# ska-telescope/ska-sdp-screen-fitting

Measured on AMD Instinct MI355X. Metric: screen-slots/sec (ant×time×freq) + FITS-cube wall-clock, KL 256² screen, higher is better.
Workload: dtype f64

## Files before the change

### include/screenfit.h

```cpp
#ifndef SCREENFIT_H
#define SCREENFIT_H

#include <stddef.h>
#include <stdint.h>

#ifdef __cplusplus
extern "C" {
#endif

#define SF_OK 0
#define SF_EINVAL (-22)
#define SF_ENOMEM (-12)
#define SF_EIO (-5)
#define SF_ENODEV (-19)

#define SF_MAX_DIR 60
#define SF_MAX_FIT_DIR 128
#define SF_MAX_EVAL_DIR 128

#define SF_SCREEN_PHASE 0
#define SF_SCREEN_TEC 1
#define SF_SCREEN_AMPLITUDE 2

#define SF_EVAL_NAN_SCRUB 1u
// ... 48 lines not shown
#define SF_EVAL_KERNEL_LDS16 4
#define SF_EVAL_KERNEL_LDS8H 5
#define SF_EVAL_KERNEL_LDS16H 6
#define SF_EVAL_KERNEL_TILE3 7
#define SF_EVAL_KERNEL_SHB 8
#define SF_EVAL_KERNEL_WIDE 9
int sf_get_eval_kernel(sf_ctx* ctx, int gain, unsigned flags, int* kernel);
#define SF_EVAL_CONTRACTION_F64 0
#define SF_EVAL_CONTRACTION_I8_DIGITS 1
int sf_get_eval_contraction(sf_ctx* ctx, int gain, unsigned flags, int* contraction);
int sf_set_option(sf_ctx* ctx, int option, int value);
int sf_alloc(sf_ctx* ctx, size_t bytes, void** dev_ptr);
int sf_free(sf_ctx* ctx, void* dev_ptr);
int sf_copy_h2d(sf_ctx* ctx, void* dst_dev, const void* src_host, size_t bytes);
int sf_copy_d2h(sf_ctx* ctx, void* dst_host, const void* src_dev, size_t bytes);

int sf_set_basis(sf_ctx* ctx, const double* pp_host, int D, double r0,
                 double beta);
int sf_set_basis_wide(sf_ctx* ctx, const double* pp_host, int D, double r0,
                      double beta);
int sf_get_basis(sf_ctx* ctx, double* c_host, double* pinv_c_host,
                 double* u_host, double* eig_host);

int sf_set_piercepoints(sf_ctx* ctx, const double* pp_host, int D, double r0,
                        double beta);

int sf_kl_fit(sf_ctx* ctx, const double* phase, const float* weight, int T,
              int F, int A, const int* station_order_host,
              const sf_fit_params* params, double* coef, double* resid,
              float* w_out, int32_t* order_out);

int sf_get_fit_stats(sf_ctx* ctx, int* n_masks, int* n_general);

int sf_get_fit_pool(sf_ctx* ctx, uint64_t* masks_host, double* entries_host,
                    int max_masks, int* n_masks);

int sf_set_grid(sf_ctx* ctx, const double* x_host, int nx,
                const double* y_host, int ny);

int sf_kl_eval(sf_ctx* ctx, const double* coef, int64_t S, float* out,
               int64_t ring_slots, unsigned flags);

int sf_kl_eval_gain(sf_ctx* ctx, const double* coef_phase,
                    const double* coef_xx, const double* coef_yy, int64_t S,
                    float* out, int64_t ring_slots, unsigned flags);
int sf_kl_eval_sums(sf_ctx* ctx, const double* coef_phase,
                    const double* coef_xx, const double* coef_yy, int64_t S,
                    float* out, int64_t ring, unsigned flags,
                    uint32_t* slot_sums);

int sf_tess_fill(sf_ctx* ctx, const int32_t* labels, int nx, int ny,
                 const double* phase, const double* amp_xx,
                 const double* amp_yy, int D, int64_t S, float* out,
                 int64_t ring_slots, double smooth_pix, unsigned flags);

int sf_smooth(sf_ctx* ctx, float* cube, int nx, int ny, int64_t n_img,
              double smooth_pix, unsigned flags);

#ifdef __cplusplus
}
#endif
#endif
```

### ska-sdp-screen-fitting_amd/csrc/capi.hip

```cpp
#include <hip/hip_runtime.h>

#include <cmath>
#include <cstring>
#include <string>
#include <vector>

#include "sf_internal.h"

namespace sf {
static thread_local std::string g_last_error;
void set_error(const std::string& msg) { g_last_error = msg; }
}

using sf::set_error;

namespace {

int check_device(int device) {
  int n = 0;
  hipError_t e = hipGetDeviceCount(&n);
  if (e != hipSuccess || n == 0) {
    set_error("no HIP device available");
    return SF_ENODEV;
  }
// ... 131 lines not shown
    std::vector<uint32_t> mask((n_cu + 31) / 32, 0u);
    for (int c = 0; c < n_cu; ++c) mask[c >> 5] |= 1u << (c & 31);
    for (int k = 0; k < n_reserve; ++k) {
      const int c = reserve_cus[k];
      SF_REQUIRE(c >= 0 && c < n_cu, SF_EINVAL, "sf_stream_create: CU index out of range");
      mask[c >> 5] &= ~(1u << (c & 31));
    }
    SF_REQUIRE(n_reserve < n_cu, SF_EINVAL, "sf_stream_create: no CU left");
    SF_HIP(hipExtStreamCreateWithCUMask(&s, (uint32_t)mask.size(), mask.data()));
  }
  *stream = s;
  return SF_OK;
}

int sf_stream_destroy(sf_ctx* ctx, void* stream) {
  SF_REQUIRE(ctx && stream, SF_EINVAL, "sf_stream_destroy: bad argument");
  SF_HIP(hipSetDevice(ctx->device));
  SF_HIP(hipStreamDestroy(reinterpret_cast<hipStream_t>(stream)));
  return SF_OK;
}

int sf_set_option(sf_ctx* ctx, int option, int value) {
  SF_REQUIRE(ctx, SF_EINVAL, "sf_set_option: NULL context");
  switch (option) {
    case SF_OPT_FIT_GENERAL:
      ctx->force_general = value != 0;
      return SF_OK;
    case SF_OPT_EVAL_KERNEL:
      SF_REQUIRE(value >= SF_EVAL_KERNEL_AUTO && value <= SF_EVAL_KERNEL_WIDE,
                 SF_EINVAL, "sf_set_option: unknown evaluation kernel");
      ctx->eval_kernel = value;
      return SF_OK;
    case SF_OPT_FIT_PACK:
      ctx->fit_pack = value != 0;
      return SF_OK;
    case SF_OPT_FIT_LEAN:
      ctx->fit_lean = value != 0;
      return SF_OK;
    case SF_OPT_EVAL_KS_PAD:
      SF_REQUIRE(value >= 0 && value <= 3, SF_EINVAL,
                 "sf_set_option: k-step padding must be 0..3");
      ctx->eval_ks_pad = value;
      return SF_OK;
    case SF_OPT_EVAL_SLEEP:
      SF_REQUIRE(value >= 0 && value <= 1000, SF_EINVAL,
                 "sf_set_option: eval sleep must be 0..1000");
      ctx->eval_sleep = value;
      return SF_OK;
    case SF_OPT_EVAL_XCD_MAP:
      SF_REQUIRE(value >= -1 && value <= 1, SF_EINVAL,
                 "sf_set_option: XCD map must be -1, 0 or 1");
      ctx->eval_xcd_map = value;
      return SF_OK;
    case SF_OPT_EVAL_GROUPS:
      SF_REQUIRE(value >= 0 && value <= 256 && (value & (value - 1)) == 0,
                 SF_EINVAL, "sf_set_option: groups must be 0 or a power of two <= 256");
      ctx->eval_groups = value;
      return SF_OK;
    case SF_OPT_EVAL_BANDS:
      SF_REQUIRE(value >= 0 && value <= 128 && (value & (value - 1)) == 0,
                 SF_EINVAL, "sf_set_option: bands must be 0 or a power of two <= 128");
      ctx->eval_bands = value;
      return SF_OK;
    case SF_OPT_TESS_SLOTS:
      SF_REQUIRE(value >= 0 && value <= 256, SF_EINVAL,
                 "sf_set_option: tess slots must be 0..256");
      ctx->tess_slots = value;
// ... 232 lines not shown
               SF_EINVAL,
               "sf_kl_fit: reference station not in this shard and no "
               "ref_phase given");
  }
  for (int a = 0; a < A; ++a)
    SF_REQUIRE(st_order[a] >= 0, SF_EINVAL, "sf_kl_fit: negative order");
  SF_HIP(hipSetDevice(ctx->device));
  if (ctx->skip_cap < (size_t)F * A) {
    SF_TRY(dev_alloc(&ctx->d_skip, (size_t)F * A));
    ctx->skip_cap = (size_t)F * A;
  }
  if (ctx->st_order_cap < (size_t)A) {
    SF_TRY(dev_alloc(&ctx->d_st_order, (size_t)A));
    ctx->st_order_cap = (size_t)A;
  }
  SF_HIP(hipMemcpyAsync(ctx->d_st_order, st_order, sizeof(int) * A,
                        hipMemcpyHostToDevice, ctx->stream));
  return sf::launch_fit(ctx, phase, weight, T, F, A, p, coef, resid, w_out,
                        order_out);
}

int sf_get_fit_stats(sf_ctx* ctx, int* n_masks, int* n_general) {
  SF_REQUIRE(ctx, SF_EINVAL, "sf_get_fit_stats: NULL context");
  int c[4] = {0, 0, 0, 0};
  SF_HIP(hipSetDevice(ctx->device));
  SF_HIP(hipStreamSynchronize(ctx->stream));
  if (ctx->d_counters)
    SF_HIP(hipMemcpy(c, ctx->d_counters, sizeof(c), hipMemcpyDeviceToHost));
  if (n_masks) *n_masks = c[0];
  if (n_general) *n_general = c[2];
  return SF_OK;
}

int sf_get_fit_pool(sf_ctx* ctx, uint64_t* masks_host, double* entries_host,
                    int max_masks, int* n_masks) {
  SF_REQUIRE(ctx && n_masks && max_masks >= 0, SF_EINVAL, "sf_get_fit_pool: bad argument");
  SF_REQUIRE(max_masks == 0 || (masks_host && entries_host), SF_EINVAL,
             "sf_get_fit_pool: NULL output");
  SF_REQUIRE(!ctx->wide, SF_EINVAL,
             "sf_get_fit_pool: no mask pool above SF_MAX_DIR directions "
             "(sf_set_basis_wide: every flagged slot decomposes its own subset)");
  SF_HIP(hipSetDevice(ctx->device));
  SF_HIP(hipStreamSynchronize(ctx->stream));
  int c0 = 0;
  if (ctx->d_counters)
    SF_HIP(hipMemcpy(&c0, ctx->d_counters, sizeof(int), hipMemcpyDeviceToHost));
  const int n = ctx->pool_D == ctx->D && (size_t)c0 <= ctx->pool_cap ? c0 : 0;
  *n_masks = n;
  const int k = n < max_masks ? n : max_masks;
  if (k > 0) {
    const size_t entry = (size_t)ctx->D * ctx->D + ctx->D;
    SF_HIP(hipMemcpy(masks_host, ctx->d_pool_mask, k * sizeof(uint64_t),
                     hipMemcpyDeviceToHost));
    SF_HIP(hipMemcpy(entries_host, ctx->d_pool, k * entry * sizeof(double),
                     hipMemcpyDeviceToHost));
  }
  return SF_OK;
}

int sf_set_grid(sf_ctx* ctx, const double* x, int nx, const double* y,
                int ny) {
  SF_REQUIRE(ctx && ctx->D > 0, SF_EINVAL,
             "sf_set_grid: call sf_set_basis or sf_set_piercepoints first");
  SF_REQUIRE(x && y && nx >= 1 && ny >= 1, SF_EINVAL, "sf_set_grid: bad grid");
  for (int i = 0; i < nx; ++i)
    SF_REQUIRE(std::isfinite(x[i]), SF_EINVAL, "sf_set_grid: non-finite x coordinate");
// ... 203 lines not shown
```

### ska-sdp-screen-fitting_amd/csrc/kl_fit_fast.hip

```cpp
#include <hip/hip_runtime.h>

#include <algorithm>
#include <cmath>
#include <cstdlib>

#include "sf_internal.h"
#include "sf_wave.h"

namespace sf {

constexpr double kAtol = 1e-3;
constexpr size_t kLdsBytes = 160 * 1024;
constexpr double kTinyW = 1e-3 * 1.001;
constexpr unsigned long long kEmptyKey = 0ull;

__host__ __device__ inline int ldo(int n) { return n | 1; }

__device__ __forceinline__ unsigned long long mix64(unsigned long long x) {
  x ^= x >> 30;
  x *= 0xbf58476d1ce4e5b9ull;
  x ^= x >> 27;
  x *= 0x94d049bb133111ebull;
  x ^= x >> 31;
  return x;
// ... 18 lines not shown
    const unsigned long long k = keys[h];
    if (k == key) return h;
    if (k == kEmptyKey) return -1;
    h = (h + 1) & (cap - 1);
  }
  return -1;
}

__device__ __forceinline__ double phase_ref(const double* phase,
                                            const double* refph, int sub,
                                            int64_t s, int a, int A, int D,
                                            int d) {
  double v = phase[s * D + d];
  if (refph) v -= refph[(s / A) * D + d];
  else if (sub >= 0) v -= phase[(s + (sub - a)) * D + d];
  return v;
}

template <int GW>
__global__ __launch_bounds__(256) void kl_classify_kernel(
    const float* __restrict__ weight, int64_t S, int F, int A, int D,
    const int* __restrict__ st_order, const uint8_t* __restrict__ skip,
    int ref_skip, unsigned long long* __restrict__ keys, int cap,
    int* __restrict__ pos, uint8_t* __restrict__ cls,
    int* __restrict__ counters,
    double* __restrict__ coef, double* __restrict__ resid,
    float* __restrict__ w_out, int32_t* __restrict__ order_out) {
  constexpr int kPerWave = 64 / GW;
  const int l = lane();
  const int g = l / GW;
  const int d = l % GW;
  const int64_t s = ((int64_t)blockIdx.x * (blockDim.x / 64) + threadIdx.x / 64) *
                        kPerWave + g;
  const bool live = s < S && d < D;
  float x = 0.0f;
  if (live) {
    x = weight[s * D + d];
    w_out[s * D + d] = x;
  }
  const unsigned long long bm = __ballot(live && x > 0.0f);
  const unsigned long long bt = __ballot(live && x > 0.0f && (double)x <= kTinyW);
  const unsigned long long gmask = (GW == 64) ? ~0ull : ((1ull << GW) - 1ull);
  const unsigned long long mask = (bm >> (g * GW)) & gmask;
  const bool tiny = ((bt >> (g * GW)) & gmask) != 0ull;
  const float w_first = __shfl(x, g * GW + (mask ? __builtin_ctzll(mask) : 0));
  const unsigned long long bn = __ballot(live && x > 0.0f && x != w_first);
  const bool nonuniform = ((bn >> (g * GW)) & gmask) != 0ull;
  if (s >= S) return;
  const int a = (int)(s % A);
  const int f = (int)((s / A) % F);
  if (live && (a == ref_skip || skip[f * A + a])) {
    coef[s * D + d] = 0.0;
    resid[s * D + d] = 0.0;
  }
  if (d != 0) return;
  if (a == ref_skip || skip[f * A + a]) {
    cls[s] = 1;
    order_out[s] = 0;
    pos[s] = -2;
    return;
  }
  order_out[s] = st_order[a];
  if (tiny) atomicAdd(counters + 2, 1);
  else if (nonuniform) atomicAdd(counters + 4, 1);
  cls[s] = tiny ? 2 : 0;
  const unsigned long long full = (D == 64) ? ~0ull : ((1ull << D) - 1ull);
  if (mask == full) pos[s] = -1;
  else if (mask == 0ull) pos[s] = -2;
  else pos[s] = table_insert(keys, cap, mask);
}

__global__ __launch_bounds__(256) void kl_assign_kernel(
    const unsigned long long* __restrict__ keys, int cap, int* __restrict__ ids,
    unsigned long long* __restrict__ pool_mask, int pool_cap,
    int* __restrict__ counters, int D) {
  int lvl = 0;
  for (int i = blockIdx.x * blockDim.x + threadIdx.x; i - lane() < cap;
       i += gridDim.x * blockDim.x) {
    const unsigned long long k = i < cap ? keys[i] : kEmptyKey;
    const bool fresh = k != kEmptyKey && ids[i] < 0;
    const unsigned long long nb = __ballot(fresh);
// ... 359 lines not shown
        const double w = fabs(lam[k]);
        r2 += (w > v) || (w == v && k < l);
      }
      perm[r2] = l;
    }
    lds_sync();
    double* e = pool + (size_t)id * (D * D + D);
    if (l < m) {
      for (int r = 0; r < m; ++r) e[l * D + r] = U[l * ld + perm[r]];
      e[D * D + l] = lam[perm[l]];
    }
    if (l == 0) status[id] = 0;
    lds_sync();
  }
}

struct FastLds {
  const double* U;
  const double* C;
  int cld;
  const double* lam;
  double* Vs;
  double* lams;
  double* G;
  double* M;
  double* vec;
  double2* cs;
  int2* pr;
};

__host__ __device__ inline size_t fast_shared_bytes(int D, bool c_global) {
  return (size_t)((c_global ? 1 : 2) * D * ldo(D) + 64) * sizeof(double);
}
__host__ __device__ inline size_t fast_wave_bytes(int D, bool slow, bool lean = false) {
  if (lean) return (size_t)6 * 64 * sizeof(double);
  return (size_t)((slow ? 3 : 2) * D * ldo(D) + 64 + 6 * 64) * sizeof(double) +
         (slow ? 64 * sizeof(double2) + 96 * sizeof(int2) : 0);
}

struct Basis {
  int n;
  bool full;
  int ld;
  const double* U;
  const double* lam;
};

__device__ __noinline__ void nl_sincos(double x, double* s, double* c) { sincos(x, s, c); }
__device__ __noinline__ double nl_atan2(double y, double x) { return atan2(y, x); }
__device__ __noinline__ double nl_log10(double x) { return log10(x); }
__device__ __noinline__ double nl_pow(double x, double y) { return pow(x, y); }
__device__ __noinline__ double nl_log(double x) { return log(x); }
__device__ __noinline__ double nl_fmod(double x, double y) { return fmod(x, y); }

template <bool NI>
struct FitMath {
  static __device__ __forceinline__ void sin_cos(double x, double* s, double* c) {
    if constexpr (NI) nl_sincos(x, s, c); else sincos(x, s, c);
  }
  static __device__ __forceinline__ double arctan2(double y, double x) {
    if constexpr (NI) return nl_atan2(y, x); else return atan2(y, x);
  }
  static __device__ __forceinline__ double lg10(double x) {
    if constexpr (NI) return nl_log10(x); else return log10(x);
  }
  static __device__ __forceinline__ double power(double x, double y) {
    if constexpr (NI) return nl_pow(x, y); else return pow(x, y);
  }
  static __device__ __forceinline__ double ln(double x) {
    if constexpr (NI) return nl_log(x); else return log(x);
  }
  static __device__ __forceinline__ double mod(double x, double y) {
    if constexpr (NI) return nl_fmod(x, y); else return fmod(x, y);
  }
};

template <bool NI = false>
__device__ __forceinline__ double model_value(int screen_type, double x) {
  return screen_type == SF_SCREEN_AMPLITUDE ? FitMath<NI>::power(10.0, x) : x;
}

template <bool SLOW, int SPW, bool LEAN>
__device__ void fit_once(const FastLds& L, const Basis& B, int D, int ld,
                         int K, int screen_type, bool uniform, double wu,
                         double phi_p, double w_p, double phi_d, double w_d,
                         double& white_d, double& resid_d) {
#pragma clang fp contract(off)
  using G = Group<SPW>;
  using M = FitMath<!SLOW>;
  constexpr bool NI = !SLOW;
  constexpr int kMatVecUnroll = LEAN ? 4 : 1;
  const int l = G::lane();
  const int n = B.n;
  double* v0 = L.vec;
  double* v1 = L.vec + 64;
  double* v2 = L.vec + 128;
  double* v3 = L.vec + 192;
  double rc = 0.0, rs = 0.0;
  if (l < n) {
    if (screen_type == SF_SCREEN_PHASE) {
      double sn, cn;
      M::sin_cos(phi_p, &sn, &cn);
      rc = w_p * cn;
      rs = w_p * sn;
    } else if (screen_type == SF_SCREEN_AMPLITUDE) {
      rc = w_p * M::lg10(phi_p);
    } else {
      rc = w_p * phi_p;
    }
    v0[l] = rc;
    v1[l] = rs;
    v2[l] = w_p;
  }
  lds_sync();
  const bool tie2 = n == 2 && K == 1;
  double t_re = 0.0, t_im = 0.0;
  if (tie2) {
    const double w2 = v2[1];
    const double iw = w2 > kAtol ? 1.0 / w2 : 0.0;
    t_re = iw * v0[1];
    t_im = iw * v1[1];
  }
  double a1 = 0.0, a2 = 0.0;
  if (l < K) {
#pragma unroll kMatVecUnroll
    for (int p = 0; p < n; ++p) {
      const double u = B.U[p * B.ld + l];
      a1 += u * v0[p];
      a2 += u * v1[p];
    }
// ... 155 lines not shown
template <bool SLOW, int SPW, bool LEAN>
__global__ __launch_bounds__(256, SLOW ? 1 : SF_FIT_MINW) void kl_fit_pass_kernel(
    int it, int niter, int64_t S, int F, int A, int D,
    const double* __restrict__ phase, const double* __restrict__ refph,
    int ref_sub, const double* __restrict__ g_u, const double* __restrict__ g_c,
    const double* __restrict__ g_eig, const int* __restrict__ st_order,
    const uint8_t* __restrict__ cls, int* __restrict__ pos,
    const int* __restrict__ ids, unsigned long long* __restrict__ keys, int cap,
    const double* __restrict__ pool, int pool_cap, int* __restrict__ counters,
    int screen_type, double nsigma, int adjust_order, double* __restrict__ coef,
    double* __restrict__ resid, float* __restrict__ w_out,
    int32_t* __restrict__ order_out) {
#pragma clang fp contract(off)
  extern __shared__ double smem[];
  const int ld = ldo(D);
  using G = Group<SPW>;
  using M = FitMath<!SLOW>;
  constexpr bool NI = !SLOW;
  constexpr bool CG = SPW == 1;
  const int nwaves = blockDim.x / 64;
  const int nslots = nwaves * SPW;
  const int wv = (threadIdx.x / 64) * SPW + G::index();
  const int d = G::lane();
  double* sU = smem;
  double* sC = CG ? nullptr : sU + D * ld;
  double* sl = sU + (CG ? 1 : 2) * D * ld;
  for (int e = threadIdx.x; e < D * D; e += blockDim.x) {
    const int r = e / D, c = e % D;
    sU[r * ld + c] = g_u[e];
    if (!CG) sC[r * ld + c] = g_c[e];
  }
  for (int e = threadIdx.x; e < 64; e += blockDim.x) sl[e] = e < D ? g_eig[e] : 0.0;
  __syncthreads();
  FastLds L;
  L.U = sU;
  L.C = CG ? g_c : sC;
  L.cld = CG ? D : ld;
  L.lam = sl;
  double* wb = sl + 64 + (size_t)wv * (fast_wave_bytes(D, SLOW, LEAN) / sizeof(double));
  if (LEAN) {
    L.Vs = L.G = L.M = L.lams = nullptr;
    L.vec = wb;
    L.cs = nullptr;
    L.pr = nullptr;
  } else {
    L.Vs = wb;
    L.G = wb + D * ld;
    L.M = L.G + D * ld;
    L.lams = (SLOW ? L.M + D * ld : L.G + D * ld);
    L.vec = L.lams + 64;
    L.cs = reinterpret_cast<double2*>(L.vec + 6 * 64);
    L.pr = reinterpret_cast<int2*>(L.cs + 64);
  }
  const uint8_t want = SLOW ? 2 : 0;

  for (int64_t s = (int64_t)blockIdx.x * nslots + wv; s < S;
       s += (int64_t)gridDim.x * nslots) {
    if (SLOW && cls[s] != want) continue;
    const uint8_t cl = SLOW ? want : cls[s];
    const int a = (int)(s % A);
    const int p0 = pos[s];
    const int64_t base = s * D;
    double phi_d = 0.0, w_d = 0.0, white_d = 0.0, resid_d = 0.0;
    if (d < D) {
      phi_d = phase_ref(phase, refph, ref_sub, s, a, A, D, d);
      w_d = (double)w_out[base + d];
      white_d = it == 0 ? 0.0 : coef[base + d];
      resid_d = it == 0 ? 0.0 : resid[base + d];
    }
    double order = (double)order_out[s];
    const double station_order = (double)st_order[a];
    if (cl != want) continue;
    int id = -1;
    if (p0 >= 0) {
      id = ids[p0];
      if (id < 0 || id >= pool_cap) {
        if (d == 0) atomicOr(counters + 3, 1);
        continue;
      }
    } else if (p0 == -3) {
      if (d == 0) atomicOr(counters + 3, 2);
      continue;
    }
    const bool unfl = (d < D) && (w_d > 0.0);
    const unsigned long long um = G::ballot(unfl);
    const int n_unfl = __popcll(um);

    Basis B;
    B.n = n_unfl;
    B.full = (n_unfl == D);
    B.ld = ld;
    if (B.full) {
      B.U = L.U;
      B.lam = L.lam;
    } else if (n_unfl > 0) {
      const double* e = pool + (size_t)id * (D * D + D);
      if (LEAN) {
        B.U = e;
        B.ld = D;
        B.lam = e + D * D;
      } else {
        for (int r = 0; r < n_unfl; ++r)
          if (d < n_unfl) L.Vs[r * ld + d] = e[r * D + d];
        if (d < n_unfl) L.lams[d] = e[D * D + d];
        lds_sync();
        B.U = L.Vs;
        B.lam = L.lams;
      }
    }
    double phi_p = 0.0, w_p = 0.0;
    {
      double* v4 = L.vec + 256;
      double* v5 = L.vec + 320;
      if (unfl) {
        const int p = G::rank(um);
        v4[p] = phi_d;
        v5[p] = w_d;
      }
      lds_sync();
      if (d < n_unfl) {
        phi_p = v4[d];
        w_p = v5[d];
      }
      lds_sync();
    }
    const double wmax = G::max(unfl ? w_d : -INFINITY);
    const double wmin = -G::max(unfl ? -w_d : -INFINITY);
    const bool uniform = (wmax == wmin);
    if (LEAN && n_unfl > 0 && !uniform) {
      if (d == 0) atomicOr(counters + 3, 4);
      continue;
    }

    if (n_unfl > 0) {
      if (order > n_unfl - 1) order = n_unfl - 1;
      if (it == 0) {
        fit_once<SLOW, SPW, LEAN>(L, B, D, ld, (int)order, screen_type, uniform, wmin,
                       phi_p, w_p, phi_d, w_d, white_d, resid_d);
      } else if (adjust_order) {
        bool hit_upper = false, hit_lower = false, hit_upper2 = false,
             hit_lower2 = false;
        double sign = 1.0, prev_redchi2 = 0.0;
        for (int oi = 0; oi < 4; ++oi) {
          if (oi > 0)
            fit_once<SLOW, SPW, LEAN>(L, B, D, ld, (int)order, screen_type, uniform, wmin,
                           phi_p, w_p, phi_d, w_d, white_d, resid_d);
// ... 234 lines not shown
    const size_t shm = (size_t)2 * subset_rows(D) * subset_ld(D) * sizeof(double) +
                       64 * sizeof(double2) + 96 * sizeof(int2) +
                       128 * sizeof(int);
    const int blocks = n_new < 8192 ? n_new : 8192;
    const int nw = ctx->fit_eig_waves > 0 ? ctx->fit_eig_waves : kEigWavesDefault;
#define SF_LAUNCH_EIG(NW)                                                              \
  do {                                                                                 \
    if (shm > 64 * 1024)                                                               \
      SF_HIP(hipFuncSetAttribute(reinterpret_cast<const void*>(&kl_subset_eig_kernel<NW>), \
                                 hipFuncAttributeMaxDynamicSharedMemorySize, (int)shm)); \
    hipLaunchKernelGGL(kl_subset_eig_kernel<NW>, dim3(blocks), dim3(64 * NW), shm,     \
                       ctx->stream, ctx->d_c, D, ctx->d_pool_mask, (int)ctx->pool_cap, \
                       ctx->d_counters, ctx->d_pool, done);                            \
  } while (0)
    switch (nw) {
      case 1: SF_LAUNCH_EIG(1); break;
      case 2: SF_LAUNCH_EIG(2); break;
      case 4: SF_LAUNCH_EIG(4); break;
      default: SF_LAUNCH_EIG(3); break;
    }
#undef SF_LAUNCH_EIG
    SF_HIP(hipGetLastError());
  }
  return SF_OK;
}

template <bool SLOW, int SPW, bool LEAN>
static int launch_pass_spw(sf_ctx* ctx, int it, const sf_fit_params* p,
                           const RefSpec& r, int64_t S, int F, int A,
                           const double* phase, double* coef, double* resid,
                           float* w_out, int32_t* order_out) {
  const int D = ctx->D;
  const size_t shared = fast_shared_bytes(D, SPW == 1);
  const size_t slot = fast_wave_bytes(D, SLOW, LEAN);
  int nw = 1, best = 0;
  for (int k = 1; k <= 4; ++k) {
    const size_t per_wg = shared + (size_t)k * SPW * slot;
    if (per_wg > kLdsBytes) break;
    const int waves = k * (int)(kLdsBytes / per_wg);
    if (waves > best) {
      best = waves;
      nw = k;
    }
  }
  const size_t shm = shared + (size_t)nw * SPW * slot;
  if (shm > 64 * 1024)
    SF_HIP(hipFuncSetAttribute(
        reinterpret_cast<const void*>(&kl_fit_pass_kernel<SLOW, SPW, LEAN>),
        hipFuncAttributeMaxDynamicSharedMemorySize, (int)shm));
  int64_t blocks = (S + nw * SPW - 1) / (nw * SPW);
  if (blocks > 16384) blocks = 16384;
  hipLaunchKernelGGL((kl_fit_pass_kernel<SLOW, SPW, LEAN>), dim3((unsigned)blocks),
                     dim3(64 * nw), shm, ctx->stream, it, p->niter, S, F, A, D,
                     phase, r.refph, r.sub, ctx->d_u, ctx->d_c, ctx->d_eig,
                     ctx->d_st_order, ctx->d_class, ctx->d_pos, ctx->d_ids,
                     ctx->d_keys, (int)ctx->table_cap, ctx->d_pool,
                     (int)ctx->pool_cap, ctx->d_counters, p->screen_type,
                     p->nsigma, p->adjust_order, coef, resid, w_out, order_out);
  SF_HIP(hipGetLastError());
  return SF_OK;
}

template <bool SLOW>
static int launch_pass(sf_ctx* ctx, int it, const sf_fit_params* p,
                       const RefSpec& r, int64_t S, int F, int A,
                       const double* phase, double* coef, double* resid,
                       float* w_out, int32_t* order_out, bool lean) {
  const bool pack = !SLOW && ctx->D <= 32 && ctx->fit_pack;
  if (!SLOW && lean && ctx->fit_lean) {
    if (pack)
      return launch_pass_spw<false, 2, true>(ctx, it, p, r, S, F, A, phase, coef,
                                             resid, w_out, order_out);
    return launch_pass_spw<false, 1, true>(ctx, it, p, r, S, F, A, phase, coef,
                                           resid, w_out, order_out);
  }
  if (pack)
    return launch_pass_spw<SLOW, 2, false>(ctx, it, p, r, S, F, A, phase, coef,
                                           resid, w_out, order_out);
  return launch_pass_spw<SLOW, 1, false>(ctx, it, p, r, S, F, A, phase, coef, resid,
                                         w_out, order_out);
}

int launch_block_sigma(sf_ctx* ctx, int T, int F, int A, const double* phase,
                       const RefSpec& r, int screen_type, const double* resid,
                       const float* w_out) {
  hipLaunchKernelGGL(kl_block_sigma_kernel, dim3(F * A), dim3(256), 0,
                     ctx->stream, T, F, A, ctx->D, phase, r.refph, r.sub,
                     ctx->d_skip, r.skip, screen_type, resid, w_out,
                     ctx->d_sigma);
  SF_HIP(hipGetLastError());
  return SF_OK;
}

int launch_fit(sf_ctx* ctx, const double* phase, const float* weight, int T,
               int F, int A, const sf_fit_params* p, double* coef,
               double* resid, float* w_out, int32_t* order_out) {
  if (ctx->wide)
    return launch_fit_wide(ctx, phase, weight, T, F, A, p, coef, resid, w_out,
                           order_out);
  const int D = ctx->D;
  const int64_t S = (int64_t)T * F * A;
  const RefSpec r = ref_spec(p, A);
  SF_TRYF(launch_skip(ctx, phase, weight, T, F, A, r));

  static const char* env = std::getenv("SCREENFIT_FIT");
  if (ctx->force_general || (env && env[0] == 'g')) {
    if (p->screen_type == SF_SCREEN_AMPLITUDE ||
        (p->niter > 1 && p->screen_type != SF_SCREEN_PHASE)) {
      set_error("the general fit kernel handles phase (any niter) and tec (niter 1) only");
      return SF_EINVAL;
    }
    return launch_fit_general(ctx, nullptr, nullptr, S, phase, weight, T, F, A,
                              p, r, coef, resid, w_out, order_out);
  }
  if (!resid) {
    SF_TRYF(grow(&ctx->d_scratch, ctx->scratch_cap, (size_t)S * D));
    resid = ctx->d_scratch;
  }
  if (!w_out || !order_out) {
    size_t wc = 0, oc = 0;
    if (ctx->d_wscratch) (void)hipFree(ctx->d_wscratch);
    if (ctx->d_oscratch) (void)hipFree(ctx->d_oscratch);
    ctx->d_wscratch = nullptr;
    ctx->d_oscratch = nullptr;
    SF_TRYF(grow(&ctx->d_wscratch, wc, (size_t)S * D));
    SF_TRYF(grow(&ctx->d_oscratch, oc, (size_t)S));
    if (!w_out) w_out = ctx->d_wscratch;
    if (!order_out) order_out = ctx->d_oscratch;
  }
// ... 7 lines not shown
    SF_TRYF(grow(&ctx->d_class, c3, (size_t)S));
    ctx->slot_cap = (size_t)S;
  }
  if (ctx->sigma_cap < (size_t)F * A) {
    size_t c = 0;
    if (ctx->d_sigma) (void)hipFree(ctx->d_sigma);
    ctx->d_sigma = nullptr;
    SF_TRYF(grow(&ctx->d_sigma, c, (size_t)F * A));
    ctx->sigma_cap = (size_t)F * A;
  }
  const size_t tcap = next_pow2((size_t)(2 * p->niter + 2) * (size_t)S + 64);
  if (ctx->table_cap < tcap) {
    size_t c1 = 0, c2 = 0;
    if (ctx->d_keys) (void)hipFree(ctx->d_keys);
    if (ctx->d_ids) (void)hipFree(ctx->d_ids);
    ctx->d_keys = nullptr;
    ctx->d_ids = nullptr;
    SF_TRYF(grow(&ctx->d_keys, c1, tcap));
    SF_TRYF(grow(&ctx->d_ids, c2, tcap));
    ctx->table_cap = tcap;
  }
  if (!ctx->d_counters) {
    size_t c = 0;
    SF_TRYF(grow(&ctx->d_counters, c, 8));
  }
  SF_TRYF(ensure_pool(ctx, 1024));
  const int cap = (int)ctx->table_cap;
  SF_HIP(hipMemsetAsync(ctx->d_keys, 0, ctx->table_cap * sizeof(unsigned long long),
                        ctx->stream));
  SF_HIP(hipMemsetAsync(ctx->d_ids, 0xff, ctx->table_cap * sizeof(int), ctx->stream));
  SF_HIP(hipMemsetAsync(ctx->d_counters, 0, 8 * sizeof(int), ctx->stream));

  {
    const int gw = D <= 8 ? 8 : D <= 16 ? 16 : D <= 32 ? 32 : 64;
    const int64_t per_block = 4 * (64 / gw);
    const dim3 grid((unsigned)((S + per_block - 1) / per_block));
#define SF_CLASSIFY(W)                                                          \
  hipLaunchKernelGGL(kl_classify_kernel<W>, grid, dim3(256), 0, ctx->stream,    \
                     weight, S, F, A, D, ctx->d_st_order, ctx->d_skip, r.skip,  \
                     ctx->d_keys, cap, ctx->d_pos, ctx->d_class,               \
                     ctx->d_counters, coef, resid, w_out, order_out)
    switch (gw) {
      case 8: SF_CLASSIFY(8); break;
      case 16: SF_CLASSIFY(16); break;
      case 32: SF_CLASSIFY(32); break;
      default: SF_CLASSIFY(64); break;
    }
#undef SF_CLASSIFY
    SF_HIP(hipGetLastError());
  }

  const bool block_flags = p->screen_type != SF_SCREEN_PHASE;
  for (int it = 0; it < p->niter; ++it) {
    int n_slow = 0, n_nonuniform = 0;
    SF_TRYF(number_and_decompose(ctx, &n_slow, &n_nonuniform));
    SF_TRYF(launch_pass<false>(ctx, it, p, r, S, F, A, phase, coef, resid,
                               w_out, order_out, n_nonuniform == 0));
    if (n_slow > 0)
      SF_TRYF(launch_pass<true>(ctx, it, p, r, S, F, A, phase, coef, resid,
                                w_out, order_out, false));
    if (block_flags && it + 1 < p->niter) {
      SF_TRYF(launch_block_sigma(ctx, T, F, A, phase, r, p->screen_type, resid,
                                 w_out));
      hipLaunchKernelGGL(kl_block_flag_kernel, dim3((unsigned)((S + 255) / 256)),
                         dim3(256), 0, ctx->stream, S, F, A, D, phase, r.refph,
                         r.sub, ctx->d_class, p->screen_type, p->nsigma,
                         ctx->d_sigma, resid, w_out, ctx->d_keys, cap,
                         ctx->d_pos);
      SF_HIP(hipGetLastError());
    }
  }
  int err = 0;
  SF_HIP(hipMemcpyAsync(&err, ctx->d_counters + 3, sizeof(int),
                        hipMemcpyDeviceToHost, ctx->stream));
  SF_HIP(hipStreamSynchronize(ctx->stream));
  SF_REQUIRE((err & 3) == 0, SF_EIO, "sf_kl_fit: internal mask table overflow");
  SF_REQUIRE((err & 4) == 0, SF_EIO,
// ... 10 lines not shown
```

### ska-sdp-screen-fitting_amd/csrc/sf_internal.h

```cpp
#pragma once

#include <hip/hip_runtime.h>

#include <cstdint>
#include <string>

#include "screenfit.h"

namespace sf {

void set_error(const std::string& msg);

#define SF_HIP(call)                                                        \
  do {                                                                      \
    hipError_t e_ = (call);                                                 \
    if (e_ != hipSuccess) {                                                 \
      ::sf::set_error(std::string(#call) + ": " + hipGetErrorString(e_));   \
      return SF_EIO;                                                        \
    }                                                                       \
  } while (0)

#define SF_REQUIRE(cond, code, msg) \
  do {                              \
    if (!(cond)) {                  \
// ... 87 lines not shown
  size_t pool_status_cap = 0;
  int pool_D = 0;
  int* d_pos = nullptr;
  uint8_t* d_class = nullptr;
  double* d_sigma = nullptr;
  size_t sigma_cap = 0;
  size_t slot_cap = 0;
  int* d_counters = nullptr;
  double* d_scratch = nullptr;
  size_t scratch_cap = 0;
  float* d_wscratch = nullptr;
  int32_t* d_oscratch = nullptr;
  double* d_gw = nullptr;
  size_t gw_cap = 0;
  double gw_sigma = -1.0;
  float* d_trash = nullptr;
  float* d_smooth = nullptr;
  size_t smooth_cap = 0;
  float* d_tess_tab = nullptr;
  size_t tess_tab_cap = 0;
  int force_general = 0;
  int eval_kernel = SF_EVAL_KERNEL_AUTO;
  int64_t eval_max_blocks = 0;
  int eval_ks_pad = 0;
  int eval_sleep = 0;
  int eval_xcd_map = -1;
  int eval_groups = 0;
  int eval_bands = 0;
  int tess_slots = 0;
  int tess_waves = 0;
  int tess_tile = 0;
  int tess_box = -1;
  int fit_pack = 1;
  int fit_lean = 1;
};

namespace sf {
constexpr int kEvalMaxKS = 15;
constexpr int kEvalWideMaxKS = SF_MAX_EVAL_DIR / 4;
inline bool eval_int_applies(const sf_ctx* ctx, bool gain, unsigned flags,
                             bool out_aligned16) {
  return !gain && ctx->dig_ok && ctx->d_cdig && ctx->eval_int != 0 &&
         (flags & SF_EVAL_FAST_SINCOS) && ctx->n_pix % 4 == 0 && out_aligned16 &&
         ctx->ksteps >= 12 && ctx->ksteps <= kEvalMaxKS;
}

struct RefSpec {
  int sub = -1;
  const double* refph = nullptr;
  int skip = -1;
};
RefSpec ref_spec(const sf_fit_params* p, int A);
int launch_skip(sf_ctx* ctx, const double* phase, const float* weight, int T,
                int F, int A, const RefSpec& r);
int launch_fit_general(sf_ctx* ctx, const int* slot_list, const int* n_list,
                       int64_t max_slots, const double* phase,
                       const float* weight, int T, int F, int A,
                       const sf_fit_params* p, const RefSpec& r, double* coef,
                       double* resid, float* w_out, int32_t* order_out);
int launch_basis(sf_ctx* ctx);
int launch_block_sigma(sf_ctx* ctx, int T, int F, int A, const double* phase,
                       const RefSpec& r, int screen_type, const double* resid,
                       const float* w_out);
int launch_basis_wide(sf_ctx* ctx);
int launch_fit_wide(sf_ctx* ctx, const double* phase, const float* weight,
                    int T, int F, int A, const sf_fit_params* p, double* coef,
// ... 27 lines not shown
```

### ska-sdp-screen-fitting_amd/csrc/sf_wave.h

```cpp
#pragma once

#include <hip/hip_runtime.h>

namespace sf {

__device__ __forceinline__ int lane() { return __lane_id(); }

__device__ __forceinline__ void lds_sync() {
  asm volatile("s_waitcnt lgkmcnt(0)" ::: "memory");
}

__device__ __forceinline__ double wave_sum(double v) {
#pragma unroll
  for (int o = 32; o > 0; o >>= 1) v += __shfl_xor(v, o, 64);
  return v;
}

__device__ __forceinline__ double wave_max(double v) {
#pragma unroll
  for (int o = 32; o > 0; o >>= 1) v = fmax(v, __shfl_xor(v, o, 64));
  return v;
}

__device__ __forceinline__ double bcast(double v, int src) {
  return __shfl(v, src, 64);
}

template <int SPW>
struct Group {
  static constexpr int kWidth = 64 / SPW;
  __device__ static int lane() { return __lane_id() & (kWidth - 1); }
  __device__ static int first() { return __lane_id() & ~(kWidth - 1); }
  __device__ static int index() { return __lane_id() / kWidth; }
  __device__ static double sum(double v) {
#pragma unroll
    for (int o = kWidth / 2; o > 0; o >>= 1) v += __shfl_xor(v, o, 64);
    return v;
  }
  __device__ static double max(double v) {
#pragma unroll
    for (int o = kWidth / 2; o > 0; o >>= 1) v = fmax(v, __shfl_xor(v, o, 64));
    return v;
  }
  __device__ static double bcast(double v, int src) {
    return __shfl(v, first() + src, 64);
  }
  __device__ static unsigned long long ballot(bool x) {
    const unsigned long long m = __ballot(x);
    if (SPW == 1) return m;
    return (m >> first()) & ((1ull << kWidth) - 1);
  }
  __device__ static bool any(bool x) { return ballot(x) != 0ull; }
  __device__ static int rank(unsigned long long m) {
    if (SPW == 1)
      return __builtin_amdgcn_mbcnt_hi((uint32_t)(m >> 32),
                                       __builtin_amdgcn_mbcnt_lo((uint32_t)m, 0));
    return __popcll(m & ((1ull << lane()) - 1));
  }
};

__device__ __forceinline__ int rr_partner(int i, int r, int m) {
  const int mm = m - 1;
  if (i == mm) return r;
  if (i == r) return mm;
  int p = 2 * r - i;
  if (p < 0) p += mm;
  if (p >= mm) p -= mm;
  return p;
}

__device__ inline int wave_jacobi(double* a, double* v, double2* cs, int2* pr,
                                  int n, int ld, int max_sweeps) {
#pragma clang fp contract(off)
  const int i = lane();
// ... 285 lines not shown
```

### ska-sdp-screen-fitting_amd/ska_sdp_screen_fitting_amd/_lib.py

```python

import contextlib
import ctypes
import os
import threading

import numpy as np

_HERE = os.path.dirname(os.path.abspath(__file__))
LIB_PATH = os.environ.get("SCREENFIT_LIB", os.path.join(_HERE, "libscreenfit.so"))

SF_SCREEN_PHASE = 0
SF_SCREEN_TEC = 1
SF_SCREEN_AMPLITUDE = 2
SF_EVAL_NAN_SCRUB = 1
SF_EVAL_FAST_SINCOS = 1 << 8
SF_EVAL_NT_STORES = 1 << 9
SF_EVAL_BIG_ENDIAN = 1 << 10
SF_MAX_DIR = 60
SF_MAX_FIT_DIR = 128
SF_MAX_EVAL_DIR = 128
SF_OPT_FIT_GENERAL = 1
SF_OPT_EVAL_KERNEL = 2
SF_OPT_EVAL_MAX_BLOCKS = 3
SF_OPT_FIT_PACK = 4
# ... 4 lines not shown
SF_OPT_EVAL_BANDS = 9
SF_OPT_FIT_LEAN = 10
SF_OPT_TESS_SLOTS = 11
SF_OPT_TESS_WAVES = 12
SF_OPT_TESS_TILE = 13
SF_OPT_TESS_BOX = 14
SF_OPT_EVAL_INT = 15
SF_OPT_EVAL_WG_WAVES = 16
SF_OPT_FIT_EIG_WAVES = 17
SF_OPT_FIT_SUBSET_DELETION = 18
SF_EVAL_KERNEL_AUTO = 0
SF_EVAL_KERNEL_TILE = 1
SF_EVAL_KERNEL_LDS4 = 2
SF_EVAL_KERNEL_LDS8 = 3
SF_EVAL_KERNEL_LDS16 = 4
SF_EVAL_KERNEL_LDS8H = 5
SF_EVAL_KERNEL_LDS16H = 6
SF_EVAL_KERNEL_TILE3 = 7
SF_EVAL_KERNEL_SHB = 8
SF_EVAL_KERNEL_WIDE = 9
EVAL_KERNEL_NAMES = {SF_EVAL_KERNEL_TILE: "kl_eval_kernel",
                     SF_EVAL_KERNEL_LDS4: "kl_eval_lds_kernel<4 waves>",
                     SF_EVAL_KERNEL_LDS8: "kl_eval_lds_kernel<8 waves>",
                     SF_EVAL_KERNEL_LDS16: "kl_eval_lds_kernel<16 waves>",
                     SF_EVAL_KERNEL_LDS8H: "kl_eval_lds_kernel<8 waves, 2 tiles>",
                     SF_EVAL_KERNEL_LDS16H: "kl_eval_lds_kernel<16 waves, 2 tiles>",
                     SF_EVAL_KERNEL_TILE3: "kl_eval_kernel<3 waves/SIMD>",
                     SF_EVAL_KERNEL_SHB: "kl_eval_kernel<Cpix in LDS>",
                     SF_EVAL_KERNEL_WIDE: "kl_eval_wide_kernel"}

EXPORTED = (
    "sf_version", "sf_last_error", "sf_create", "sf_destroy", "sf_set_stream",
    "sf_synchronize", "sf_set_option", "sf_get_eval_kernel", "sf_get_eval_contraction", "sf_alloc", "sf_free", "sf_copy_h2d", "sf_copy_d2h",
    "sf_set_basis", "sf_set_basis_wide", "sf_set_piercepoints", "sf_get_basis", "sf_kl_fit", "sf_get_fit_stats", "sf_get_fit_pool",
    "sf_stream_create", "sf_stream_destroy", "sf_device_cus",
    "sf_set_grid", "sf_kl_eval", "sf_kl_eval_gain", "sf_kl_eval_sums",
    "sf_tess_fill", "sf_smooth",
)


_identity = {}


def library_identity(path=None):
    import hashlib
    p = os.path.realpath(path or LIB_PATH)
    if p not in _identity:
        h = hashlib.sha256()
        with open(p, "rb") as fh:
            for blk in iter(lambda: fh.read(1 << 20), b""):
                h.update(blk)
        _identity[p] = {"sha16": h.hexdigest()[:16], "bytes": os.path.getsize(p)}
    return dict(_identity[p])


class ScreenFitError(RuntimeError):
    """Raised for any failure of the HIP library (including its absence)."""


class FitParams(ctypes.Structure):
    _fields_ = [("screen_type", ctypes.c_int), ("niter", ctypes.c_int),
                ("nsigma", ctypes.c_double), ("adjust_order", ctypes.c_int),
                ("ref_ant", ctypes.c_int), ("ant_offset", ctypes.c_int),
                ("ref_phase", ctypes.c_void_p)]


_lib = None
# ... 6 lines not shown
        if _lib is not None and path is None:
            return _lib
        p = path or LIB_PATH
        if not os.path.exists(p):
            raise ScreenFitError(
                f"libscreenfit.so not found at {p}: build it with "
                "`make -C ska-sdp-screen-fitting_amd/csrc` (or "
                "__graft_entry__.build()); there is no CPU fallback")
        lib = ctypes.CDLL(p)
        vp, ip, c_int, c_dbl = (ctypes.c_void_p, ctypes.POINTER(ctypes.c_int),
                                ctypes.c_int, ctypes.c_double)
        i64 = ctypes.c_int64
        sig = {
            "sf_version": ([], ctypes.c_char_p),
            "sf_last_error": ([], ctypes.c_char_p),
            "sf_create": ([c_int, ctypes.POINTER(vp)], c_int),
            "sf_destroy": ([vp], c_int),
            "sf_set_stream": ([vp, vp], c_int),
            "sf_synchronize": ([vp], c_int),
            "sf_set_option": ([vp, c_int, c_int], c_int),
            "sf_get_eval_kernel": ([vp, c_int, ctypes.c_uint, ip], c_int),
            "sf_get_eval_contraction": ([vp, c_int, ctypes.c_uint, ip], c_int),
            "sf_alloc": ([vp, ctypes.c_size_t, ctypes.POINTER(vp)], c_int),
            "sf_free": ([vp, vp], c_int),
            "sf_copy_h2d": ([vp, vp, vp, ctypes.c_size_t], c_int),
            "sf_copy_d2h": ([vp, vp, vp, ctypes.c_size_t], c_int),
            "sf_set_basis": ([vp, vp, c_int, c_dbl, c_dbl], c_int),
            "sf_set_basis_wide": ([vp, vp, c_int, c_dbl, c_dbl], c_int),
            "sf_set_piercepoints": ([vp, vp, c_int, c_dbl, c_dbl], c_int),
            "sf_get_basis": ([vp, vp, vp, vp, vp], c_int),
            "sf_kl_fit": ([vp, vp, vp, c_int, c_int, c_int, ip,
                           ctypes.POINTER(FitParams), vp, vp, vp, vp], c_int),
            "sf_get_fit_stats": ([vp, ip, ip], c_int),
            "sf_get_fit_pool": ([vp, vp, vp, c_int, ip], c_int),
            "sf_set_grid": ([vp, vp, c_int, vp, c_int], c_int),
            "sf_kl_eval": ([vp, vp, i64, vp, i64, ctypes.c_uint], c_int),
            "sf_stream_create": ([vp, ctypes.POINTER(c_int), c_int,
                                  ctypes.POINTER(vp)], c_int),
            "sf_stream_destroy": ([vp, vp], c_int),
            "sf_device_cus": ([vp, ctypes.POINTER(c_int)], c_int),
            "sf_kl_eval_gain": ([vp, vp, vp, vp, i64, vp, i64, ctypes.c_uint],
                                c_int),
            "sf_kl_eval_sums": ([vp, vp, vp, vp, i64, vp, i64, ctypes.c_uint, vp],
                                c_int),
            "sf_tess_fill": ([vp, vp, c_int, c_int, vp, vp, vp, c_int, i64, vp,
                              i64, c_dbl, ctypes.c_uint], c_int),
            "sf_smooth": ([vp, vp, c_int, c_int, i64, c_dbl, ctypes.c_uint], c_int),
        }
        for name, (args, res) in sig.items():
            fn = getattr(lib, name)
            fn.argtypes = args
            fn.restype = res
        if path is None:
            _lib = lib
        return lib


def _check(rc, what):
    if rc != 0:
        msg = load_library().sf_last_error().decode(errors="replace")
        raise ScreenFitError(f"{what} failed ({rc}): {msg}")


_TORCH_DTYPES = {np.float64: "torch.float64", np.float32: "torch.float32",
                 np.int32: "torch.int32", np.int64: "torch.int64"}

# ... 104 lines not shown
        c, pinv, u = (np.empty((D, D)) for _ in range(3))
        eig = np.empty(D)
        _check(self.lib.sf_get_basis(self.h, c.ctypes.data, pinv.ctypes.data,
                                     u.ctypes.data, eig.ctypes.data),
               "sf_get_basis")
        return c, pinv, u, eig

    def fit(self, phase, weight, T, F, A, station_order, screen_type=0,
            niter=2, nsigma=5.0, adjust_order=True, ref_ant=-1, coef=None,
            resid=None, w_out=None, order_out=None, ant_offset=0,
            ref_phase=None):
        so = np.ascontiguousarray(station_order, dtype=np.int32)
        if so.shape != (A,):
            raise ValueError(f"station_order: shape {so.shape}, expected ({A},)")
        n = int(T) * int(F) * int(A) * self.D
        prm = FitParams(int(screen_type), int(niter), float(nsigma),
                        int(bool(adjust_order)), int(ref_ant), int(ant_offset),
                        self._dev(ref_phase, np.float64, int(T) * int(F) * self.D,
                             "ref_phase"))
        _check(self.lib.sf_kl_fit(
            self.h, self._dev(phase, np.float64, n, "phase"),
            self._dev(weight, np.float32, n, "weight"), int(T), int(F), int(A),
            so.ctypes.data_as(ctypes.POINTER(ctypes.c_int)),
            ctypes.byref(prm), self._dev(coef, np.float64, n, "coef"),
            self._dev(resid, np.float64, n, "resid"),
            self._dev(w_out, np.float32, n, "w_out"),
            self._dev(order_out, np.int32, n // max(self.D, 1), "order_out")),
            "sf_kl_fit")

    def fit_stats(self):
        nm, ng = ctypes.c_int(), ctypes.c_int()
        _check(self.lib.sf_get_fit_stats(self.h, ctypes.byref(nm), ctypes.byref(ng)),
               "sf_get_fit_stats")
        return {"n_masks": nm.value, "n_general": ng.value}

    def fit_pool(self):
        n = ctypes.c_int(0)
        _check(self.lib.sf_get_fit_pool(self.h, None, None, 0, ctypes.byref(n)),
               "sf_get_fit_pool")
        D = self.D
        masks = np.zeros(n.value, np.uint64)
        ent = np.zeros((n.value, D * D + D))
        if n.value:
            _check(self.lib.sf_get_fit_pool(self.h, masks.ctypes.data, ent.ctypes.data,
                                            n.value, ctypes.byref(n)), "sf_get_fit_pool")
        order = np.argsort(masks, kind="stable")
        masks, ent = masks[order], ent[order]
        for k, m in enumerate(masks):
            n = bin(int(m)).count("1")
            u = ent[k, :D * D].reshape(D, D)
            u[n:, :] = 0.0
            u[:, n:] = 0.0
            ent[k, D * D + n:] = 0.0
        return masks, ent

    def set_grid(self, x, y):
        x = np.ascontiguousarray(x, dtype=np.float64)
        y = np.ascontiguousarray(y, dtype=np.float64)
        _check(self.lib.sf_set_grid(self.h, x.ctypes.data, x.size,
                                    y.ctypes.data, y.size), "sf_set_grid")
        self.grid = (x.size, y.size)

    def _out_numel(self, S, ring):
        nx, ny = self.grid if self.grid else (0, 0)
        return min(int(S), ring) * 4 * nx * ny

    def eval(self, coef, S, out, ring_slots=None,
# ... 110 lines not shown
```

Baseline: 6.335 million.

## Pack more fit slots per wavefront with D-dependent group widths

```diff
diff --git a/include/screenfit.h b/include/screenfit.h
--- a/include/screenfit.h
+++ b/include/screenfit.h
@@ -104,6 +104,8 @@
 
 int sf_get_fit_stats(sf_ctx* ctx, int* n_masks, int* n_general);
 
+int sf_get_fit_pack(sf_ctx* ctx, int* slots_per_wave);
+
 int sf_get_fit_pool(sf_ctx* ctx, uint64_t* masks_host, double* entries_host,
                     int max_masks, int* n_masks);
 
diff --git a/ska-sdp-screen-fitting_amd/csrc/capi.hip b/ska-sdp-screen-fitting_amd/csrc/capi.hip
--- a/ska-sdp-screen-fitting_amd/csrc/capi.hip
+++ b/ska-sdp-screen-fitting_amd/csrc/capi.hip
@@ -187,7 +187,9 @@
       ctx->eval_kernel = value;
       return SF_OK;
     case SF_OPT_FIT_PACK:
-      ctx->fit_pack = value != 0;
+      SF_REQUIRE(value >= 0 && value <= 2, SF_EINVAL,
+                 "sf_set_option: fit packing must be 0, 1 or 2");
+      ctx->fit_pack = value;
       return SF_OK;
     case SF_OPT_FIT_LEAN:
       ctx->fit_lean = value != 0;
@@ -486,6 +488,12 @@
   return SF_OK;
 }
 
+int sf_get_fit_pack(sf_ctx* ctx, int* slots_per_wave) {
+  SF_REQUIRE(ctx && slots_per_wave, SF_EINVAL, "sf_get_fit_pack: bad argument");
+  *slots_per_wave = ctx->fit_spw_last;
+  return SF_OK;
+}
+
 int sf_get_fit_pool(sf_ctx* ctx, uint64_t* masks_host, double* entries_host,
                     int max_masks, int* n_masks) {
   SF_REQUIRE(ctx && n_masks && max_masks >= 0, SF_EINVAL, "sf_get_fit_pool: bad argument");
diff --git a/ska-sdp-screen-fitting_amd/csrc/kl_fit_fast.hip b/ska-sdp-screen-fitting_amd/csrc/kl_fit_fast.hip
--- a/ska-sdp-screen-fitting_amd/csrc/kl_fit_fast.hip
+++ b/ska-sdp-screen-fitting_amd/csrc/kl_fit_fast.hip
@@ -74,7 +74,7 @@
   const int d = l % GW;
   const int64_t s = ((int64_t)blockIdx.x * (blockDim.x / 64) + threadIdx.x / 64) *
                         kPerWave + g;
-  const bool live = s < S && d < D;
+  const bool live = g < kPerWave && s < S && d < D;
   float x = 0.0f;
   if (live) {
     x = weight[s * D + d];
@@ -85,10 +85,11 @@
   const unsigned long long gmask = (GW == 64) ? ~0ull : ((1ull << GW) - 1ull);
   const unsigned long long mask = (bm >> (g * GW)) & gmask;
   const bool tiny = ((bt >> (g * GW)) & gmask) != 0ull;
-  const float w_first = __shfl(x, g * GW + (mask ? __builtin_ctzll(mask) : 0));
+  const float w_first =
+      __shfl(x, g < kPerWave ? g * GW + (mask ? __builtin_ctzll(mask) : 0) : l);
   const unsigned long long bn = __ballot(live && x > 0.0f && x != w_first);
   const bool nonuniform = ((bn >> (g * GW)) & gmask) != 0ull;
-  if (s >= S) return;
+  if (g >= kPerWave || s >= S) return;
   const int a = (int)(s % A);
   const int f = (int)((s / A) % F);
   if (live && (a == ref_skip || skip[f * A + a])) {
@@ -514,9 +515,14 @@
 __host__ __device__ inline size_t fast_shared_bytes(int D, bool c_global) {
   return (size_t)((c_global ? 1 : 2) * D * ldo(D) + 64) * sizeof(double);
 }
-__host__ __device__ inline size_t fast_wave_bytes(int D, bool slow, bool lean = false) {
-  if (lean) return (size_t)6 * 64 * sizeof(double);
-  return (size_t)((slow ? 3 : 2) * D * ldo(D) + 64 + 6 * 64) * sizeof(double) +
+__host__ __device__ constexpr int fast_vec_len(int spw) {
+  return spw == 1 ? 64 : spw <= 3 ? 32 : 64 / spw;
+}
+__host__ __device__ inline size_t fast_wave_bytes(int D, bool slow, bool lean = false,
+                                                  int vlen = 64) {
+  const int vecs = 6 * vlen + (vlen < 64 ? 2 : 0);
+  if (lean) return (size_t)vecs * sizeof(double);
+  return (size_t)((slow ? 3 : 2) * D * ldo(D) + 64 + vecs) * sizeof(double) +
          (slow ? 64 * sizeof(double2) + 96 * sizeof(int2) : 0);
 }
 
@@ -574,10 +580,11 @@
   constexpr int kMatVecUnroll = LEAN ? 4 : 1;
   const int l = G::lane();
   const int n = B.n;
+  constexpr int VL = fast_vec_len(SPW);
   double* v0 = L.vec;
-  double* v1 = L.vec + 64;
-  double* v2 = L.vec + 128;
-  double* v3 = L.vec + 192;
+  double* v1 = L.vec + VL;
+  double* v2 = L.vec + 2 * VL;
+  double* v3 = L.vec + 3 * VL;
   double rc = 0.0, rs = 0.0;
   if (l < n) {
     if (screen_type == SF_SCREEN_PHASE) {
@@ -799,12 +806,14 @@
   }
   for (int e = threadIdx.x; e < 64; e += blockDim.x) sl[e] = e < D ? g_eig[e] : 0.0;
   __syncthreads();
+  if (G::index() >= SPW) return;
   FastLds L;
   L.U = sU;
   L.C = CG ? g_c : sC;
   L.cld = CG ? D : ld;
   L.lam = sl;
-  double* wb = sl + 64 + (size_t)wv * (fast_wave_bytes(D, SLOW, LEAN) / sizeof(double));
+  constexpr int VL = fast_vec_len(SPW);
+  double* wb = sl + 64 + (size_t)wv * (fast_wave_bytes(D, SLOW, LEAN, VL) / sizeof(double));
   if (LEAN) {
     L.Vs = L.G = L.M = L.lams = nullptr;
     L.vec = wb;
@@ -816,7 +825,7 @@
     L.M = L.G + D * ld;
     L.lams = (SLOW ? L.M + D * ld : L.G + D * ld);
     L.vec = L.lams + 64;
-    L.cs = reinterpret_cast<double2*>(L.vec + 6 * 64);
+    L.cs = reinterpret_cast<double2*>(L.vec + 6 * VL);
     L.pr = reinterpret_cast<int2*>(L.cs + 64);
   }
   const uint8_t want = SLOW ? 2 : 0;
@@ -877,8 +886,8 @@
     }
     double phi_p = 0.0, w_p = 0.0;
     {
-      double* v4 = L.vec + 256;
-      double* v5 = L.vec + 320;
+      double* v4 = L.vec + 4 * VL;
+      double* v5 = L.vec + 5 * VL;
       if (unfl) {
         const int p = G::rank(um);
         v4[p] = phi_d;
@@ -1179,7 +1188,7 @@
                            float* w_out, int32_t* order_out) {
   const int D = ctx->D;
   const size_t shared = fast_shared_bytes(D, SPW == 1);
-  const size_t slot = fast_wave_bytes(D, SLOW, LEAN);
+  const size_t slot = fast_wave_bytes(D, SLOW, LEAN, fast_vec_len(SPW));
   int nw = 1, best = 0;
   for (int k = 1; k <= 4; ++k) {
     const size_t per_wg = shared + (size_t)k * SPW * slot;
@@ -1208,24 +1217,45 @@
   return SF_OK;
 }
 
+static int fit_slots_per_wave(const sf_ctx* ctx) {
+  const int D = ctx->D;
+  if (ctx->fit_pack == 0 || D > 32) return 1;
+  if (ctx->fit_pack == 2) return 2;
+  return D <= 8 ? 8 : D <= 16 ? 4 : D <= 21 ? 3 : 2;
+}
+
 template <bool SLOW>
 static int launch_pass(sf_ctx* ctx, int it, const sf_fit_params* p,
                        const RefSpec& r, int64_t S, int F, int A,
                        const double* phase, double* coef, double* resid,
                        float* w_out, int32_t* order_out, bool lean) {
-  const bool pack = !SLOW && ctx->D <= 32 && ctx->fit_pack;
-  if (!SLOW && lean && ctx->fit_lean) {
-    if (pack)
-      return launch_pass_spw<false, 2, true>(ctx, it, p, r, S, F, A, phase, coef,
-                                             resid, w_out, order_out);
-    return launch_pass_spw<false, 1, true>(ctx, it, p, r, S, F, A, phase, coef,
-                                           resid, w_out, order_out);
-  }
-  if (pack)
-    return launch_pass_spw<SLOW, 2, false>(ctx, it, p, r, S, F, A, phase, coef,
-                                           resid, w_out, order_out);
-  return launch_pass_spw<SLOW, 1, false>(ctx, it, p, r, S, F, A, phase, coef, resid,
-                                         w_out, order_out);
+#define SF_PASS(SPW, LEAN)                                                      \
+  return launch_pass_spw<SLOW, SPW, LEAN>(ctx, it, p, r, S, F, A, phase, coef, \
+                                          resid, w_out, order_out)
+  if constexpr (SLOW) {
+    SF_PASS(1, false);
+  } else {
+    int spw = fit_slots_per_wave(ctx);
+    const bool lean_pass = lean && ctx->fit_lean;
+    if (!lean_pass && spw == 3) spw = 2;
+    ctx->fit_spw_last = spw;
+    if (lean_pass) {
+      switch (spw) {
+        case 8: SF_PASS(8, true);
+        case 4: SF_PASS(4, true);
+        case 3: SF_PASS(3, true);
+        case 2: SF_PASS(2, true);
+        default: SF_PASS(1, true);
+      }
+    }
+    switch (spw) {
+      case 8: SF_PASS(8, false);
+      case 4: SF_PASS(4, false);
+      case 2: SF_PASS(2, false);
+      default: SF_PASS(1, false);
+    }
+  }
+#undef SF_PASS
 }
 
 int launch_block_sigma(sf_ctx* ctx, int T, int F, int A, const double* phase,
@@ -1242,6 +1272,7 @@
 int launch_fit(sf_ctx* ctx, const double* phase, const float* weight, int T,
                int F, int A, const sf_fit_params* p, double* coef,
                double* resid, float* w_out, int32_t* order_out) {
+  ctx->fit_spw_last = 1;
   if (ctx->wide)
     return launch_fit_wide(ctx, phase, weight, T, F, A, p, coef, resid, w_out,
                            order_out);
@@ -1315,7 +1346,8 @@
   SF_HIP(hipMemsetAsync(ctx->d_counters, 0, 8 * sizeof(int), ctx->stream));
 
   {
-    const int gw = D <= 8 ? 8 : D <= 16 ? 16 : D <= 32 ? 32 : 64;
+    const int gw = D <= 8 ? 8 : D <= 16 ? 16
+                 : fit_slots_per_wave(ctx) == 3 ? 21 : D <= 32 ? 32 : 64;
     const int64_t per_block = 4 * (64 / gw);
     const dim3 grid((unsigned)((S + per_block - 1) / per_block));
 #define SF_CLASSIFY(W)                                                          \
@@ -1326,6 +1358,7 @@
     switch (gw) {
       case 8: SF_CLASSIFY(8); break;
       case 16: SF_CLASSIFY(16); break;
+      case 21: SF_CLASSIFY(21); break;
       case 32: SF_CLASSIFY(32); break;
       default: SF_CLASSIFY(64); break;
     }
diff --git a/ska-sdp-screen-fitting_amd/csrc/sf_internal.h b/ska-sdp-screen-fitting_amd/csrc/sf_internal.h
--- a/ska-sdp-screen-fitting_amd/csrc/sf_internal.h
+++ b/ska-sdp-screen-fitting_amd/csrc/sf_internal.h
@@ -143,6 +143,7 @@
   int tess_tile = 0;
   int tess_box = -1;
   int fit_pack = 1;
+  int fit_spw_last = 1;
   int fit_lean = 1;
 };
 
diff --git a/ska-sdp-screen-fitting_amd/csrc/sf_wave.h b/ska-sdp-screen-fitting_amd/csrc/sf_wave.h
--- a/ska-sdp-screen-fitting_amd/csrc/sf_wave.h
+++ b/ska-sdp-screen-fitting_amd/csrc/sf_wave.h
@@ -29,17 +29,49 @@
 template <int SPW>
 struct Group {
   static constexpr int kWidth = 64 / SPW;
-  __device__ static int lane() { return __lane_id() & (kWidth - 1); }
-  __device__ static int first() { return __lane_id() & ~(kWidth - 1); }
+  static constexpr bool kPow2 = (kWidth & (kWidth - 1)) == 0;
+  static_assert(SPW == 1 || kWidth <= 32, "groups are at most half a wave");
+  static_assert(kPow2 || kWidth > 16, "the partner rule needs p ^ 16 < kWidth");
   __device__ static int index() { return __lane_id() / kWidth; }
+  __device__ static int first() {
+    return kPow2 ? (__lane_id() & ~(kWidth - 1)) : index() * kWidth;
+  }
+  __device__ static int lane() {
+    return kPow2 ? (__lane_id() & (kWidth - 1)) : __lane_id() - first();
+  }
+  __device__ static int partner(int o) {
+    int p = lane() ^ o;
+    if (p >= kWidth) p ^= 16;
+    return first() + p;
+  }
   __device__ static double sum(double v) {
-#pragma unroll
-    for (int o = kWidth / 2; o > 0; o >>= 1) v += __shfl_xor(v, o, 64);
+    if (kPow2) {
+#pragma unroll
+      for (int o = 16; o >= kWidth && SPW > 1; o >>= 1) v += 0.0;
+#pragma unroll
+      for (int o = kWidth / 2; o > 0; o >>= 1) v += __shfl_xor(v, o, 64);
+    } else {
+      const int l = lane();
+      const double x = __shfl(v, first() + ((l ^ 16) < kWidth ? (l ^ 16) : l), 64);
+      v += (l ^ 16) < kWidth ? x : 0.0;
+#pragma unroll
+      for (int o = 8; o > 0; o >>= 1) v += __shfl(v, partner(o), 64);
+    }
     return v;
   }
   __device__ static double max(double v) {
-#pragma unroll
-    for (int o = kWidth / 2; o > 0; o >>= 1) v = fmax(v, __shfl_xor(v, o, 64));
+    if (kPow2) {
+#pragma unroll
+      for (int o = 16; o >= kWidth && SPW > 1; o >>= 1) v = fmax(v, -INFINITY);
+#pragma unroll
+      for (int o = kWidth / 2; o > 0; o >>= 1) v = fmax(v, __shfl_xor(v, o, 64));
+    } else {
+      const int l = lane();
+      const double x = __shfl(v, first() + ((l ^ 16) < kWidth ? (l ^ 16) : l), 64);
+      v = fmax(v, (l ^ 16) < kWidth ? x : -INFINITY);
+#pragma unroll
+      for (int o = 8; o > 0; o >>= 1) v = fmax(v, __shfl(v, partner(o), 64));
+    }
     return v;
   }
   __device__ static double bcast(double v, int src) {
diff --git a/ska-sdp-screen-fitting_amd/ska_sdp_screen_fitting_amd/_lib.py b/ska-sdp-screen-fitting_amd/ska_sdp_screen_fitting_amd/_lib.py
--- a/ska-sdp-screen-fitting_amd/ska_sdp_screen_fitting_amd/_lib.py
+++ b/ska-sdp-screen-fitting_amd/ska_sdp_screen_fitting_amd/_lib.py
@@ -60,7 +60,7 @@
 EXPORTED = (
     "sf_version", "sf_last_error", "sf_create", "sf_destroy", "sf_set_stream",
     "sf_synchronize", "sf_set_option", "sf_get_eval_kernel", "sf_get_eval_contraction", "sf_alloc", "sf_free", "sf_copy_h2d", "sf_copy_d2h",
-    "sf_set_basis", "sf_set_basis_wide", "sf_set_piercepoints", "sf_get_basis", "sf_kl_fit", "sf_get_fit_stats", "sf_get_fit_pool",
+    "sf_set_basis", "sf_set_basis_wide", "sf_set_piercepoints", "sf_get_basis", "sf_kl_fit", "sf_get_fit_stats", "sf_get_fit_pack", "sf_get_fit_pool",
     "sf_stream_create", "sf_stream_destroy", "sf_device_cus",
     "sf_set_grid", "sf_kl_eval", "sf_kl_eval_gain", "sf_kl_eval_sums",
     "sf_tess_fill", "sf_smooth",
@@ -133,6 +133,7 @@
             "sf_kl_fit": ([vp, vp, vp, c_int, c_int, c_int, ip,
                            ctypes.POINTER(FitParams), vp, vp, vp, vp], c_int),
             "sf_get_fit_stats": ([vp, ip, ip], c_int),
+            "sf_get_fit_pack": ([vp, ip], c_int),
             "sf_get_fit_pool": ([vp, vp, vp, c_int, ip], c_int),
             "sf_set_grid": ([vp, vp, c_int, vp, c_int], c_int),
             "sf_kl_eval": ([vp, vp, i64, vp, i64, ctypes.c_uint], c_int),
@@ -303,7 +304,10 @@
         nm, ng = ctypes.c_int(), ctypes.c_int()
         _check(self.lib.sf_get_fit_stats(self.h, ctypes.byref(nm), ctypes.byref(ng)),
                "sf_get_fit_stats")
-        return {"n_masks": nm.value, "n_general": ng.value}
+        spw = ctypes.c_int()
+        _check(self.lib.sf_get_fit_pack(self.h, ctypes.byref(spw)), "sf_get_fit_pack")
+        return {"n_masks": nm.value, "n_general": ng.value,
+                "slots_per_wave": spw.value}
 
     def fit_pool(self):
         n = ctypes.c_int(0)
```

Result: no change. 6.361 million, median of 6 (+0.4%).
